# zhyever/PatchRefinerV2

Measured on AMD Instinct MI355X. Metric: 4K depth maps/sec (cai-mode r32), higher is better.
Workload: dtype bf16x3+f16f6; 1 GPU; v2_zoe_4k_r32; model=PatchRefinerPlus, cai_mode=r32, patches_per_frame=81, coarse_branch=ZoeDepth/DPT_BEiT_L_384, max_batch=41, streams=3, hip_graph=False, prefetch_next_coarse=True, frames=torch.rand, seeded, weights=synthetic (numpy PCG64 keyed by parameter name)

## Files before the change

patchrefinerv2_amd/csrc/conv3x3_f6.hip:

```cpp
#include <cstdlib>
#include <type_traits>

#include "igemm.h"
#include "conv3x3_gate_epi.h"

namespace prv2 {

namespace f6 {
constexpr int TH = 8, TW = 16, HW_ = TW + 2, HALO = (TH + 2) * HW_;
constexpr int PIX = 288;
constexpr int A_BYTES = HALO * PIX;
constexpr int ST_CHUNK = 1040, ST_DMAS = 6, ST_WAVE = ST_DMAS * ST_CHUNK;
constexpr int ST_BASE = 2 * A_BYTES;
constexpr int LDS_BYTES = ST_BASE + 8 * ST_WAVE;
constexpr int STEP_BYTES = 8 * 2 * 4 * 1024;
#ifndef F6_D
#define F6_D 4
#endif
constexpr int D = F6_D;
#ifndef F6_CV0
#define F6_CV0 2
#endif
#ifndef F6_CV1
#define F6_CV1 5
#endif
constexpr int CV_TAP0 = F6_CV0, CV_TAP1 = F6_CV1;
static_assert(LDS_BYTES <= 160 * 1024, "LDS budget");
static_assert(8 * ST_DMAS * 4 >= HALO, "staging covers the halo");
}

struct F6Params {
  const float* x;
  const char* w;
  const float* bias;
  const float* res;
  float* y;
  unsigned* range;
  int N, H, W, Cin, ldx, ldy, ld_res;
  long long x_bstride, y_bstride;
  float x_scale, out_scale;
  int relu_in, y_x2;
  long long* stamps;
};

typedef int i32x4 __attribute__((ext_vector_type(4)));
typedef int i32x8 __attribute__((ext_vector_type(8)));
typedef unsigned u32x6 __attribute__((ext_vector_type(6)));
typedef _Float16 f16x8 __attribute__((ext_vector_type(8)));

__device__ __forceinline__ u32x6 cvt_fp6(const f32x16& a, const f32x16& b, float scale) {
  u32x6 q;
  asm volatile("v_cvt_scalef32_2xpk16_fp6_f32 %0, %1, %2, %3" : "=&v"(q) : "v"(a), "v"(b), "v"(scale));
  return q;
}
__device__ __forceinline__ int e8m0_of(float m) {
  const int eb = (int)((__float_as_uint(m) >> 23) & 0xffu);
  return min(max(eb - 2, 1), 254);
}

__device__ __forceinline__ unsigned long long uniform64(unsigned long long v) {
  return (unsigned long long)(unsigned)__builtin_amdgcn_readfirstlane((int)(unsigned)v) |
         ((unsigned long long)(unsigned)__builtin_amdgcn_readfirstlane((int)(unsigned)(v >> 32)) << 32);
}

#ifndef F6_DBG_NOW
#define F6_LDW(dst, voff, sbase, imm) asm volatile("global_load_dwordx4 %0, %1, %2 offset:" #imm : "=v"(dst) : "v"(voff), "s"(sbase) : "memory")
#else
#define F6_LDW(dst, voff, sbase, imm) asm volatile("global_load_dwordx4 %0, %1, %2 offset:" #imm : "=v"(dst) : "v"(lane * 16), "s"(p.w) : "memory")
#endif

template <bool X2IN, class Epi>
__device__ __forceinline__ void f6_body(const F6Params& p, char* const smem, const int t_begin, const int per, const int K, Epi&& epi) {
  using namespace f6;
  const int tid = threadIdx.x, lane = tid & 63, wave = __builtin_amdgcn_readfirstlane(tid >> 6);
  const int m16 = lane & 15, g = lane >> 4;
  const unsigned lds0 = (unsigned)(size_t)smem;
  const int tiles_x = (p.W + TW - 1) / TW, tiles_xy = tiles_x * ((p.H + TH - 1) / TH);
  auto tile_of = [&](int k, int& n, int& y0, int& x0) {
    const int t = t_begin + k * per;
    n = t / tiles_xy;
    const int r = t - n * tiles_xy, ty = r / tiles_x;
    y0 = ty * TH;
    x0 = (r - ty * tiles_x) * TW;
  };

  constexpr unsigned OOB = 0x80000000u;
  i32x4 rsrc;
  rsrc.z = __builtin_amdgcn_readfirstlane((int)(unsigned)((((long long)p.H * p.W - 1) * p.ldx + p.Cin) * 4));
  rsrc.w = 0x00020000;
  unsigned hoff[ST_DMAS];
  auto set_loader = [&](int k) {
    int n, y0, x0;
    tile_of(k, n, y0, x0);
    const unsigned long long img_base = (unsigned long long)(size_t)(p.x + (long long)n * p.x_bstride);
    rsrc.x = __builtin_amdgcn_readfirstlane((int)(unsigned)img_base);
    rsrc.y = __builtin_amdgcn_readfirstlane((int)(unsigned)((img_base >> 32) & 0xffffu));
#pragma unroll
    for (int i = 0; i < ST_DMAS; ++i) {
      const int hp = (wave * ST_DMAS + i) * 4 + g;
      const int hy = hp / HW_, hx = hp - hy * HW_;
      const int iy = y0 - 1 + hy, ix = x0 - 1 + hx;
      const bool ok = hp < HALO && (unsigned)iy < (unsigned)p.H && (unsigned)ix < (unsigned)p.W;
      hoff[i] = ok ? (unsigned)(((iy * p.W + ix) * p.ldx + m16 * 4) * 4) : OOB;
    }
  };
  set_loader(0);
  const int nss = p.Cin >> 6, nsteps = nss * 9;
#ifdef F6_DBG_NODMA
  i32x4 dbg_sink;
#endif
  const unsigned st_wave = lds0 + ST_BASE + wave * ST_WAVE;
  auto dma_halo = [&](int ss) {
    const unsigned cofs = (unsigned)(ss * 256);
#pragma unroll
    for (int i = 0; i < ST_DMAS; ++i) {
      const unsigned dst = __builtin_amdgcn_readfirstlane(st_wave + i * ST_CHUNK);
      const unsigned voff = hoff[i] + cofs;
#ifndef F6_DBG_NODMA
      asm volatile("s_mov_b32 m0, %0\n\ts_nop 0\n\tbuffer_load_dwordx4 %1, %2, 0 offen lds" ::"s"(dst), "v"(voff), "s"(rsrc) : "memory");
#else
      asm volatile("buffer_load_dwordx4 %0, %1, %2, 0 offen" : "=v"(dbg_sink) : "v"(voff), "s"(rsrc) : "memory");
#endif
    }
  };
  const int lp = lane >> 1, cs = lane & 1, chp = wave * 24 + lp;
  const char* const st_rd = smem + ST_BASE + wave * ST_WAVE + (lp >> 2) * ST_CHUNK + (lp & 3) * 256 + cs * 128;
  const float xs = p.x_scale;
  const float relu_floor = p.relu_in ? 0.f : -__builtin_inff();
  float seen = 0.f;
  auto convert = [&](int wbuf) {
    if (lane < 48) {
      f32x16 a, b;
#pragma unroll
      for (int k = 0; k < 4; ++k) {
        f32x4 ta, tb;
        if constexpr (X2IN) {
          typedef unsigned u32x2v __attribute__((ext_vector_type(2)));
          const int q = k >> 1, h = k & 1;
          const u32x2v ah = *reinterpret_cast<const u32x2v*>(st_rd + 32 * q + 8 * h), al = *reinterpret_cast<const u32x2v*>(st_rd + 32 * q + 16 + 8 * h);
          const u32x2v bh = *reinterpret_cast<const u32x2v*>(st_rd + 64 + 32 * q + 8 * h), bl = *reinterpret_cast<const u32x2v*>(st_rd + 64 + 32 * q + 16 + 8 * h);
#pragma unroll
          for (int e = 0; e < 4; ++e) {
            const unsigned sh = (e & 1) ? 0u : 16u;
            ta[e] = __uint_as_float((ah[e >> 1] << sh) & 0xffff0000u) + __uint_as_float((al[e >> 1] << sh) & 0xffff0000u);
            tb[e] = __uint_as_float((bh[e >> 1] << sh) & 0xffff0000u) + __uint_as_float((bl[e >> 1] << sh) & 0xffff0000u);
          }
        } else {
          ta = *reinterpret_cast<const f32x4*>(st_rd + 16 * k);
          tb = *reinterpret_cast<const f32x4*>(st_rd + 64 + 16 * k);
        }
#pragma unroll
        for (int e = 0; e < 4; ++e) {
          a[4 * k + e] = fmaxf(ta[e], relu_floor) * xs;
          b[4 * k + e] = fmaxf(tb[e], relu_floor) * xs;
        }
// ... 71 lines not shown
#endif
  for (int ss = 0; ss < nss; ++ss) {
    const bool last_ss = ss + 1 == nss, more = !last_ss || k + 1 < K;
    const char* const xb = smem + ((k * nss + ss) & 1) * A_BYTES + xlane;
    auto read_item = [&](int it, int tap) {
      const int pp = it >> 3, a = it & 7, ky = tap / 3, kx = tap - 3 * ky;
      const char* q = xb + ((a + ky) * HW_ + kx) * PIX + (pp == 0 ? 0 : pp == 1 ? 64 : 128);
#ifdef F6_ABL_NOREAD
      if (k > 0 || ss > 0 || tap > 0 || it >= D) return;
#endif
      rlo[it % D] = *reinterpret_cast<const i32x4*>(q);
      if (pp == 2) rhi[it % D] = *reinterpret_cast<const i32x4*>(q + 64);
    };
    auto step = [&](auto tap_c) {
      constexpr int tap = decltype(tap_c)::value;
      constexpr int DM = tap == 0 ? ST_DMAS : 0;
      constexpr int DP = tap == 1 ? ST_DMAS : 0;
      const int s = ss * 9 + tap;
      const unsigned long long sb = uniform64(w_of(s + 1));
      if constexpr (tap == 0) {
#pragma unroll
        for (int it = 0; it < D - 1; ++it) read_item(it, 0);
      }
#pragma unroll
      for (int it = 0; it < 24; ++it) {
        const int pp = it >> 3, a = it & 7;
        if (it == 0) asm volatile("s_waitcnt vmcnt(%4)" : "+v"(wf0[0]), "+v"(wf0[1]), "+v"(wf1[0]), "+v"(wf1[1]) : "n"(6 + DP) : "memory");
        if (it == 8) asm volatile("s_waitcnt vmcnt(%2)" : "+v"(wf1[0]), "+v"(wf1[1]) : "n"(6 + DM) : "memory");
        if (it == 16) asm volatile("s_waitcnt vmcnt(%4)" : "+v"(wql[0]), "+v"(wqh[0]), "+v"(wql[1]), "+v"(wqh[1]) : "n"(4 + DM) : "memory");
        {
          const int nt = it + D - 1;
          if (nt < 24) read_item(nt, tap);
          else if (tap < 8) read_item(nt - 24, tap + 1);
        }
        __builtin_amdgcn_sched_barrier(0);
        if (pp == 0) {
          const f16x8 xf = __builtin_bit_cast(f16x8, rlo[it % D]);
          acc[a][0] = __builtin_amdgcn_mfma_f32_16x16x32_f16(__builtin_bit_cast(f16x8, wf0[0]), xf, acc[a][0], 0, 0, 0);
          acc[a][1] = __builtin_amdgcn_mfma_f32_16x16x32_f16(__builtin_bit_cast(f16x8, wf0[1]), xf, acc[a][1], 0, 0, 0);
        } else if (pp == 1) {
          const f16x8 xf = __builtin_bit_cast(f16x8, rlo[it % D]);
          acc[a][0] = __builtin_amdgcn_mfma_f32_16x16x32_f16(__builtin_bit_cast(f16x8, wf1[0]), xf, acc[a][0], 0, 0, 0);
          acc[a][1] = __builtin_amdgcn_mfma_f32_16x16x32_f16(__builtin_bit_cast(f16x8, wf1[1]), xf, acc[a][1], 0, 0, 0);
        } else {
          const i32x4 xl = rlo[it % D], xh = rhi[it % D];
          const i32x8 xq = {xl.x, xl.y, xl.z, xl.w, xh.x, xh.y, 0, 0};
          const i32x8 q0 = {wql[0].x, wql[0].y, wql[0].z, wql[0].w, wqh[0].x, wqh[0].y, 0, 0};
          const i32x8 q1 = {wql[1].x, wql[1].y, wql[1].z, wql[1].w, wqh[1].x, wqh[1].y, 0, 0};
          acc[a][0] = __builtin_amdgcn_mfma_scale_f32_16x16x128_f8f6f4(q0, xq, acc[a][0], 2, 2, 0, wqh[0].z, 0, xh.z);
          acc[a][1] = __builtin_amdgcn_mfma_scale_f32_16x16x128_f8f6f4(q1, xq, acc[a][1], 2, 2, 0, wqh[1].z, 0, xh.z);
        }
        __builtin_amdgcn_sched_barrier(0);
        if (it == 7) {
          F6_LOAD_F0(sb);
          if constexpr (tap == 0) {
            if (last_ss && k + 1 < K) set_loader(k + 1);
            dma_halo(last_ss ? (k + 1 < K ? 0 : ss) : ss + 1);
          }
#ifndef F6_ABL_NOCV
          if constexpr (tap == CV_TAP0) {
            if (more && wave < 4) convert((k * nss + ss + 1) & 1);
          }
          if constexpr (tap == CV_TAP1) {
            if (more && wave >= 4) convert((k * nss + ss + 1) & 1);
          }
#endif
        }
        if (it == 15) {
          F6_LOAD_F1(sb);
        }
        if (it == 23) F6_LOAD_Q(sb);
        __builtin_amdgcn_sched_barrier(0);
      }
    };
    step(std::integral_constant<int, 0>{});
    step(std::integral_constant<int, 1>{});
    step(std::integral_constant<int, 2>{});
    step(std::integral_constant<int, 3>{});
    step(std::integral_constant<int, 4>{});
    step(std::integral_constant<int, 5>{});
    step(std::integral_constant<int, 6>{});
    step(std::integral_constant<int, 7>{});
    step(std::integral_constant<int, 8>{});
    asm volatile("s_waitcnt lgkmcnt(0)\n\ts_barrier" ::: "memory");
  }
  {
#ifdef F6_STAMPS
    const long long st_b = __builtin_readcyclecounter();
#endif
    int n_img, y0, x0;
    tile_of(k, n_img, y0, x0);
    epi(n_img, y0, x0, acc, ((k * nss + nss - 1) & 1) * A_BYTES);
#ifdef F6_STAMPS
    const long long st_c = __builtin_readcyclecounter();
    st_main += st_b - st_a; st_epi += st_c - st_b;
#endif
  }
  }
  asm volatile("s_waitcnt vmcnt(0)" : "+v"(wf0[0]), "+v"(wf0[1]), "+v"(wf1[0]), "+v"(wf1[1]), "+v"(wql[0]), "+v"(wqh[0]), "+v"(wql[1]), "+v"(wqh[1])::"memory");
  if (p.range) {
    float m = seen;
#pragma unroll
    for (int o = 32; o > 0; o >>= 1) m = fmaxf(m, __shfl_xor(m, o, 64));
    if (lane == 0 && __float_as_uint(m) > __hip_atomic_load(p.range, __ATOMIC_RELAXED, __HIP_MEMORY_SCOPE_AGENT)) atomicMax(p.range, __float_as_uint(m));
  }
#ifdef F6_STAMPS
  if (p.stamps && lane == 0) {
    long long* o = p.stamps + ((long long)blockIdx.x * 8 + wave) * 8;
    o[0] = st_main; o[1] = st_epi; o[2] = K; o[3] = st_pro; o[4] = __builtin_readcyclecounter() - st_t0; o[5] = __builtin_amdgcn_s_memrealtime() - st_r0;
  }
#endif
}

__global__ void __launch_bounds__(512, 2) conv3x3_c256_f6_kernel(const F6Params p) {
  using namespace f6;
  __shared__ __attribute__((aligned(16))) char smem[LDS_BYTES];
  const int tiles_xy = ((p.W + TW - 1) / TW) * ((p.H + TH - 1) / TH), ntiles = p.N * tiles_xy;
  const int per = max((int)gridDim.x >> 3, 1), xcd = blockIdx.x & 7, jwg = blockIdx.x >> 3, chunk = (ntiles + 7) / 8;
  const int t_begin = xcd * chunk + jwg, t_end = min((xcd + 1) * chunk, ntiles);
  const int K = t_begin < t_end ? (t_end - t_begin + per - 1) / per : 0;
  if (K == 0) return;
  const int lane = threadIdx.x & 63, wave = __builtin_amdgcn_readfirstlane((int)threadIdx.x >> 6), m16 = lane & 15, g = lane >> 4;
  const int c0 = wave * 32 + g * 8;
  const float os = p.out_scale;
#ifndef F6_EPI_DIRECT
  constexpr int RP = 1040;
  const int tid = threadIdx.x, srow = tid >> 5, c8 = (tid & 31) * 8;
  f6_body<false>(p, smem, t_begin, per, K, [&](int n_img, int y0, int x0, f32x4 (&acc)[8][2], const int free_buf) {
    auto row_ptr = [&](int r) { return smem + (r < 48 ? ST_BASE + r * RP : free_buf + (r - 48) * RP); };
    f32x4 b0 = {0.f, 0.f, 0.f, 0.f}, b1 = b0;
    if (p.bias) {
      b0 = *reinterpret_cast<const f32x4*>(p.bias + c0);
      b1 = *reinterpret_cast<const f32x4*>(p.bias + c0 + 4);
    }
    const long long img_px = (long long)n_img * p.H * p.W;
    const __amdgpu_buffer_rsrc_t res_rs = __builtin_amdgcn_make_buffer_rsrc((void*)(p.res ? p.res + img_px * p.ld_res : p.x), 0,
                                                                            p.res ? (int)(((unsigned)(p.H * p.W - 1) * p.ld_res + 256) * 4u) : 0, 0x00020000);
    float* const ybase = p.y + (long long)n_img * p.y_bstride + c8;
#pragma unroll
    for (int h = 0; h < 2; ++h) {
      f32x4 r0[4], r1[4];
#pragma unroll
      for (int i = 0; i < 4; ++i) {
        const int iy = y0 + 4 * h + i, ixs = x0 + srow;
        const unsigned off = (iy < p.H && ixs < p.W) ? (unsigned)(((iy * p.W + ixs) * p.ld_res + c8) * 4) : 0x80000000u;
        r0[i] = __builtin_bit_cast(f32x4, __builtin_amdgcn_raw_buffer_load_b128(res_rs, off, 0, 0));
        r1[i] = __builtin_bit_cast(f32x4, __builtin_amdgcn_raw_buffer_load_b128(res_rs, off + 16, 0, 0));
      }
#pragma unroll
      for (int a = 0; a < 4; ++a) {
        char* q = row_ptr(a * TW + m16) + c0 * 4;
        *reinterpret_cast<f32x4*>(q) = acc[4 * h + a][0] * os + b0;
        *reinterpret_cast<f32x4*>(q + 16) = acc[4 * h + a][1] * os + b1;
        acc[4 * h + a][0] = acc[4 * h + a][1] = f32x4{0.f, 0.f, 0.f, 0.f};
      }
      asm volatile("s_waitcnt lgkmcnt(0)\n\ts_barrier" ::: "memory");
#pragma unroll
      for (int i = 0; i < 4; ++i) {
        const int iy = y0 + 4 * h + i, ixs = x0 + srow;
        const char* q = row_ptr(srow + 16 * i) + c8 * 4;
        const f32x4 v0 = *reinterpret_cast<const f32x4*>(q) + r0[i], v1 = *reinterpret_cast<const f32x4*>(q + 16) + r1[i];
#ifndef F6_DBG_NOEPI
        if (iy < p.H && ixs < p.W) {
          float* const dst = ybase + (long long)(iy * p.W + ixs) * p.ldy;
          if (p.y_x2) {
            bf16x4 h0, l0, h1, l1;
            split_bf16(v0, h0, l0);
            split_bf16(v1, h1, l1);
            const bf16x8 hv = __builtin_shufflevector(h0, h1, 0, 1, 2, 3, 4, 5, 6, 7), lv = __builtin_shufflevector(l0, l1, 0, 1, 2, 3, 4, 5, 6, 7);
            asm volatile("global_store_dwordx4 %0, %1, off\n\tglobal_store_dwordx4 %0, %2, off offset:16\n\ts_nop 1" ::"v"(dst), "v"(hv), "v"(lv) : "memory");
          } else {
            asm volatile("global_store_dwordx4 %0, %1, off\n\tglobal_store_dwordx4 %0, %2, off offset:16\n\ts_nop 1" ::"v"(dst), "v"(v0), "v"(v1) : "memory");
          }
        }
#endif
      }
      asm volatile("s_waitcnt lgkmcnt(0)\n\ts_barrier" ::: "memory");
    }
  });
#else
  f6_body<false>(p, smem, t_begin, per, K, [&](int n_img, int y0, int x0, f32x4 (&acc)[8][2], int) {
    f32x4 b0 = {0.f, 0.f, 0.f, 0.f}, b1 = b0;
    if (p.bias) {
      b0 = *reinterpret_cast<const f32x4*>(p.bias + c0);
      b1 = *reinterpret_cast<const f32x4*>(p.bias + c0 + 4);
    }
    const unsigned long long rb = (unsigned long long)(size_t)(p.res ? p.res + (long long)n_img * p.H * p.W * p.ld_res : p.x);
    i32x4 rr;
    rr.x = __builtin_amdgcn_readfirstlane((int)(unsigned)rb);
    rr.y = __builtin_amdgcn_readfirstlane((int)(unsigned)((rb >> 32) & 0xffffu));
    rr.z = __builtin_amdgcn_readfirstlane(p.res ? (int)(((unsigned)(p.H * p.W - 1) * p.ld_res + 256) * 4u) : 0);
    rr.w = 0x00020000;
    const int ix = x0 + m16;
    const unsigned voff = (unsigned)(((y0 * p.W + ix) * p.ld_res + c0) * 4);
    const int row = p.W * p.ld_res * 4;
    f32x4 r0[8], r1[8];
#pragma unroll
    for (int a = 0; a < 8; ++a) {
      const int so = __builtin_amdgcn_readfirstlane(a * row);
      asm volatile("buffer_load_dwordx4 %0, %2, %3, %4 offen\n\tbuffer_load_dwordx4 %1, %2, %3, %4 offen offset:16"
                   : "=&v"(r0[a]), "=&v"(r1[a]) : "v"(voff), "s"(rr), "s"(so) : "memory");
    }
    float* const ybase = p.y + (long long)n_img * p.y_bstride + c0;
#pragma unroll
    for (int a = 0; a < 8; ++a) {
      asm volatile("s_waitcnt vmcnt(%2)" : "+v"(r0[a]), "+v"(r1[a]) : "n"(2 * (7 - a)) : "memory");
      acc[a][0] = acc[a][0] * os + b0 + r0[a];
      acc[a][1] = acc[a][1] * os + b1 + r1[a];
    }
#pragma unroll
    for (int a = 0; a < 8; ++a) {
#ifndef F6_DBG_NOEPI
      if (y0 + a < p.H && ix < p.W) {
        const f32x4 v0 = acc[a][0], v1 = acc[a][1];
        float* const dst = ybase + (long long)((y0 + a) * p.W + ix) * p.ldy;
        if (p.y_x2) {
          bf16x4 h0, l0, h1, l1;
          split_bf16(v0, h0, l0);
          split_bf16(v1, h1, l1);
          const bf16x8 hv = __builtin_shufflevector(h0, h1, 0, 1, 2, 3, 4, 5, 6, 7), lv = __builtin_shufflevector(l0, l1, 0, 1, 2, 3, 4, 5, 6, 7);
          asm volatile("global_store_dwordx4 %0, %1, off\n\tglobal_store_dwordx4 %0, %2, off offset:16\n\ts_nop 1" ::"v"(dst), "v"(hv), "v"(lv) : "memory");
        } else {
          asm volatile("global_store_dwordx4 %0, %1, off\n\tglobal_store_dwordx4 %0, %2, off offset:16\n\ts_nop 1" ::"v"(dst), "v"(v0), "v"(v1) : "memory");
        }
      }
#endif
      acc[a][0] = acc[a][1] = f32x4{0.f, 0.f, 0.f, 0.f};
    }
  });
#endif
}

template <bool X2IN>
__global__ void __launch_bounds__(512, 2) conv3x3_c256_gate_f6_kernel(const GateConvParams gp) {
  using namespace f6;
  static_assert(LDS_BYTES >= g256::EPI_FLOATS * 4, "the C tile fits the main loop's LDS");
  __shared__ __attribute__((aligned(16))) char smem[LDS_BYTES];
  const IgemmParams& c = gp.c;
  F6Params p;
  p.x = c.x; p.w = reinterpret_cast<const char*>(c.w); p.bias = c.bias; p.res = nullptr; p.y = nullptr; p.range = gp.f6_range;
  p.N = c.N; p.H = c.H; p.W = c.W; p.Cin = c.Cin; p.ldx = c.ldx; p.ldy = c.ldy; p.ld_res = 0;
  p.x_bstride = c.x_bstride; p.y_bstride = c.y_bstride; p.x_scale = gp.f6_x_scale; p.out_scale = gp.f6_out_scale; p.relu_in = c.relu_in; p.y_x2 = 0;
  p.stamps = nullptr;
  int t = blockIdx.x;
  {
    const int ntiles = gridDim.x, q = ntiles >> 3, r = ntiles & 7, xcd = t & 7;
    t = (xcd < r ? xcd * (q + 1) : r * (q + 1) + (xcd - r) * q) + (t >> 3);
  }
  const int lane = threadIdx.x & 63, wave = __builtin_amdgcn_readfirstlane((int)threadIdx.x >> 6), m16 = lane & 15, g = lane >> 4;
  const int c0 = wave * 32 + g * 8;
  const float os = p.out_scale;
  PRV2_STAMP(0);
  PRV2_STAMP(1);
  PRV2_CLK_STAMP(0);
  f6_body<X2IN>(p, smem, t, 1, 1, [&](int n_img, int y0, int x0, f32x4 (&acc)[8][2], int) {
    asm volatile("s_waitcnt vmcnt(0) lgkmcnt(0)\n\ts_barrier" ::: "memory");
    PRV2_STAMP(2);
    c256_epilogue<PRV2_PREC_BF16X3, true, X2IN>(gp, reinterpret_cast<float*>(smem), n_img, y0, x0, [&](float* ct) {
      f32x4 b0 = {0.f, 0.f, 0.f, 0.f}, b1 = b0;
      if (c.bias) {
        b0 = *reinterpret_cast<const f32x4*>(c.bias + c0);
        b1 = *reinterpret_cast<const f32x4*>(c.bias + c0 + 4);
      }
#pragma unroll
      for (int a = 0; a < 8; ++a) {
        float* q = ct + (a * TW + m16) * g256::CLD + c0;
        *reinterpret_cast<f32x4*>(q) = acc[a][0] * os + b0;
        *reinterpret_cast<f32x4*>(q + 4) = acc[a][1] * os + b1;
      }
    });
  });
}

__global__ void __launch_bounds__(256) f6_pack_weight_kernel(const float* __restrict__ w, float w_scale, char* __restrict__ dst, int cin, int nsteps) {
  const int idx = blockIdx.x * blockDim.x + threadIdx.x;
  const int lane = idx & 63, j = (idx >> 6) & 1, wv = (idx >> 7) & 7, s = idx >> 10;
  if (s >= nsteps) return;
  const int ss = s / 9, tap = s - 9 * ss;
  const int r = lane & 15, g = lane >> 4;
  const int co = 32 * wv + 8 * (r >> 2) + 4 * j + (r & 3);
  const float* wr = w + (long long)co * cin * 9 + tap;
  char* o = dst + ((((long long)s * 8 + wv) * 2 + j) * 4) * 1024 + lane * 16;
#pragma unroll
  for (int part = 0; part < 2; ++part) {
    f16x8 h;
#pragma unroll
    for (int i = 0; i < 8; ++i) h[i] = (_Float16)(wr[(long long)(64 * ss + 32 * part + 8 * g + i) * 9] * w_scale);
    *reinterpret_cast<f16x8*>(o + part * 1024) = h;
  }
  f32x16 a, b;
  const int sl = g >> 1;
#pragma unroll
  for (int i = 0; i < 32; ++i) {
    const float v = wr[(long long)(64 * ss + 32 * sl + i) * 9] * w_scale;
    const float q = (g & 1) ? v : v - (float)(_Float16)v;
    if (i < 16) a[i] = q;
    else b[i - 16] = q;
  }
  float m = 0.f;
#pragma unroll
  for (int i = 0; i < 16; ++i) m = fmaxf(m, fmaxf(fabsf(a[i]), fabsf(b[i])));
  const int e = e8m0_of(m);
  const u32x6 q = cvt_fp6(a, b, __uint_as_float((unsigned)e << 23));
  typedef unsigned u32x4 __attribute__((ext_vector_type(4)));
  *reinterpret_cast<u32x4*>(o + 2 * 1024) = u32x4{q[0], q[1], q[2], q[3]};
  *reinterpret_cast<u32x4*>(o + 3 * 1024) = u32x4{q[4], q[5], (unsigned)e, 0u};
}

static inline bool aligned16(const void* q) { return (reinterpret_cast<uintptr_t>(q) & 15) == 0; }

static bool f6_shape_ok(const prv2_conv_desc* d) {
  return d->kh == 3 && d->kw == 3 && d->stride == 1 && d->pad == 1 && d->convt_k == 0 && !d->same_pad && d->cout == 256 && d->cin >= 64 &&
         d->cin % 64 == 0 && d->w >= f6::TW && (long long)d->h * d->w * d->ldx < (1LL << 29) && (long long)d->h * d->w * d->ldy < (1LL << 29);
}

}

using namespace prv2;

extern "C" int prv2_conv3x3_f6_supported(const prv2_conv_desc* d) { return d && f6_shape_ok(d) ? 1 : 0; }

extern "C" int64_t prv2_conv3x3_f6_weight_bytes(int32_t cout, int32_t cin) {
  return cout == 256 && cin >= 64 && cin % 64 == 0 ? (int64_t)(cin / 64) * 9 * f6::STEP_BYTES : 0;
}

extern "C" int prv2_pack_conv3x3_f6_weight(const float* w_src, float w_scale, void* w_packed, int32_t cout, int32_t cin, void* stream) {
  PRV2_REQUIRE(w_src && w_packed && aligned16(w_packed), "pack_conv3x3_f6_weight: null / unaligned pointer");
  PRV2_REQUIRE(prv2_conv3x3_f6_weight_bytes(cout, cin) > 0, "pack_conv3x3_f6_weight: 256 output channels, cin %% 64 == 0 (got %d -> %d)", cin, cout);
  PRV2_REQUIRE(w_scale > 0.f && (__builtin_bit_cast(unsigned, w_scale) & 0x7fffffu) == 0, "pack_conv3x3_f6_weight: w_scale is a power of two");
  const int nsteps = cin / 64 * 9;
  hipLaunchKernelGGL(f6_pack_weight_kernel, dim3((unsigned)(nsteps * 1024 / 256)), dim3(256), 0, (hipStream_t)stream, w_src, w_scale,
                     reinterpret_cast<char*>(w_packed), (int)cin, nsteps);
  PRV2_LAUNCH_CHECK("pack_conv3x3_f6_weight");
  return 0;
}

extern "C" int prv2_conv3x3_f6(const prv2_conv_desc* d, const float* x, const void* w_packed, const float* bias, const float* res, float x_scale,
                               float out_scale, uint32_t* range_word, float* y, void* stream) {
  PRV2_REQUIRE(d && x && w_packed && y, "conv3x3_f6: null pointer");
  PRV2_REQUIRE(f6_shape_ok(d), "conv3x3_f6: 3x3 s1 p1, cout 256, cin %% 64 == 0, width >= 16 (got %dx%d %d->%d k%d s%d)", d->h, d->w, d->cin, d->cout,
               d->kh, d->stride);
  PRV2_REQUIRE(d->act == PRV2_ACT_NONE && !(d->fmt & ~PRV2_FMT_Y_X2), "conv3x3_f6: no activation; the only format bit is PRV2_FMT_Y_X2");
  PRV2_REQUIRE(x_scale > 0.f && (__builtin_bit_cast(unsigned, x_scale) & 0x7fffffu) == 0 && out_scale > 0.f, "conv3x3_f6: x_scale is a power of two");
  F6Params p;
  memset(&p, 0, sizeof(p));
  p.x = x; p.w = reinterpret_cast<const char*>(w_packed); p.bias = bias; p.res = res; p.y = y; p.range = range_word;
  p.N = d->n; p.H = d->h; p.W = d->w; p.Cin = d->cin; p.ldx = d->ldx; p.ldy = d->ldy; p.ld_res = d->ld_res;
  p.x_bstride = d->x_bstride ? d->x_bstride : (long long)d->h * d->w * d->ldx;
  p.y_bstride = d->y_bstride ? d->y_bstride : (long long)d->h * d->w * d->ldy;
  p.x_scale = x_scale; p.out_scale = out_scale; p.relu_in = d->relu_in; p.y_x2 = (d->fmt & PRV2_FMT_Y_X2) != 0;
  PRV2_REQUIRE(d->n > 0 && d->h > 0 && d->ldx >= d->cin && d->ldx % 4 == 0 && aligned16(x) && p.x_bstride % 4 == 0, "conv3x3_f6: x layout");
  PRV2_REQUIRE(d->ldy >= d->cout && d->ldy % 4 == 0 && aligned16(y) && p.y_bstride % 4 == 0, "conv3x3_f6: y layout");
  PRV2_REQUIRE(!bias || aligned16(bias), "conv3x3_f6: bias alignment");
  PRV2_REQUIRE(!res || (d->ld_res >= d->cout && d->ld_res % 4 == 0 && aligned16(res) && (long long)d->h * d->w * d->ld_res < (1LL << 29)), "conv3x3_f6: res layout");
// ... 59 lines not shown
```

patchrefinerv2_amd/csrc/conv3x3_gate_epi.h:

```cpp
#pragma once
#include <cstdlib>
#include <type_traits>

#include "igemm.h"

namespace prv2 {

namespace g256 {
constexpr int BN = 256, TH = 8, TW = 16, HW_ = TW + 2;
constexpr int HALO = (TH + 2) * HW_;
constexpr int A_IT = (HALO * 8 + 511) / 512;
constexpr int A_IT2 = (HALO * 4 + 511) / 512;
constexpr int AROW = 160;
constexpr int A_BYTES = HALO * AROW, B_BYTES = BN * 128, NBUF = 3;
constexpr int CLD = BN + 4;
constexpr int ROWS = TH * TW;
constexpr int MAIN_BYTES = 2 * A_BYTES + NBUF * B_BYTES;
constexpr int EPI_FLOATS = ROWS * CLD + 2 * ROWS + 2 * BN;
constexpr int SMEM_FLOATS = MAIN_BYTES / 4 > EPI_FLOATS ? MAIN_BYTES / 4 : EPI_FLOATS;
static_assert(SMEM_FLOATS * 4 <= 160 * 1024, "LDS budget");
constexpr int NA = 4, NJ = 4, ND = 4;
}

__device__ __forceinline__ float sigmoid_fast(float v) {
// ... 270 lines not shown
  if (gp.y_x2) {
    constexpr int C8 = BN / 8, RPP8 = 512 / C8, NR8 = ROWS / RPP8;
    const int col8 = tid % C8;
    auto pix8 = [&](int i) {
      const int rr = tid / C8 + i * RPP8;
      return min(y0 + rr / TW, p.H - 1) * p.W + min(x0 + (rr & (TW - 1)), p.W - 1);
    };
    const __amdgpu_buffer_rsrc_t res_rs8 = __builtin_amdgcn_make_buffer_rsrc(
        (void*)(p.res ? p.res + (long long)n_img * p.H * p.W * p.ld_res : p.x), 0, p.res ? (int)(((unsigned)(p.H * p.W - 1) * p.ld_res + BN) * 4u) : 0,
        0x00020000);
    f32x4 rv8[NR8][2];
#pragma unroll
    for (int i = 0; i < NR8; ++i) {
      rv8[i][0] = __builtin_bit_cast(f32x4, __builtin_amdgcn_raw_buffer_load_b128(res_rs8, (pix8(i) * p.ld_res + col8 * 8) * 4, 0, 0));
      rv8[i][1] = __builtin_bit_cast(f32x4, __builtin_amdgcn_raw_buffer_load_b128(res_rs8, (pix8(i) * p.ld_res + col8 * 8 + 4) * 4, 0, 0));
    }
    float* const ybase8 = p.y + (long long)n_img * p.y_bstride + col8 * 8;
    dispatch_act(p.act, [&](auto act_c) {
#pragma unroll
      for (int i = 0; i < NR8; ++i) {
        const int rr = tid / C8 + i * RPP8;
        f32x4 v0 = *reinterpret_cast<const f32x4*>(&csm[rr * CLD + col8 * 8]), v1 = *reinterpret_cast<const f32x4*>(&csm[rr * CLD + col8 * 8 + 4]);
#pragma unroll
        for (int e = 0; e < 4; ++e) {
          v0[e] = act_apply_bf(v0[e], decltype(act_c)::value) + rv8[i][0][e];
          v1[e] = act_apply_bf(v1[e], decltype(act_c)::value) + rv8[i][1][e];
        }
        bf16x4 h0, l0, h1, l1;
        split_bf16(v0, h0, l0);
        split_bf16(v1, h1, l1);
        const bf16x8 hv = __builtin_shufflevector(h0, h1, 0, 1, 2, 3, 4, 5, 6, 7);
        const bf16x8 lv = __builtin_shufflevector(l0, l1, 0, 1, 2, 3, 4, 5, 6, 7);
        if (y0 + rr / TW < p.H && x0 + (rr & (TW - 1)) < p.W) {
          float* dst = ybase8 + (long long)pix8(i) * p.ldy;
          asm volatile("global_store_dwordx4 %0, %1, off\n\tglobal_store_dwordx4 %0, %2, off offset:16\n\ts_nop 1" ::"v"(dst), "v"(hv), "v"(lv) : "memory");
        }
      }
    });
    return;
  }
  constexpr int C4 = BN / 4, RPP = 512 / C4, NR = ROWS / RPP;
  const int col4 = tid % C4;
  auto pix_of = [&](int i) {
    const int rr = tid / C4 + i * RPP;
    return min(y0 + rr / TW, p.H - 1) * p.W + min(x0 + (rr & (TW - 1)), p.W - 1);
  };
  const __amdgpu_buffer_rsrc_t res_rs = __builtin_amdgcn_make_buffer_rsrc(
      (void*)(p.res ? p.res + (long long)n_img * p.H * p.W * p.ld_res : p.x), 0, p.res ? (int)(((unsigned)(p.H * p.W - 1) * p.ld_res + BN) * 4u) : 0,
      0x00020000);
  f32x4 rv[NR];
#pragma unroll
  for (int i = 0; i < NR; ++i) rv[i] = __builtin_bit_cast(f32x4, __builtin_amdgcn_raw_buffer_load_b128(res_rs, (pix_of(i) * p.ld_res + col4 * 4) * 4, 0, 0));
  float* const ybase = p.y + (long long)n_img * p.y_bstride + col4 * 4;
  auto store_rows = [&](auto act_c, auto ln_c) {
    constexpr bool LN = decltype(ln_c)::value;
    f32x4 lw = {1.f, 1.f, 1.f, 1.f}, lb = {0.f, 0.f, 0.f, 0.f};
    if constexpr (LN) {
      lw = *reinterpret_cast<const f32x4*>(ln_par + col4 * 4);
      lb = *reinterpret_cast<const f32x4*>(ln_par + BN + col4 * 4);
    }
#pragma unroll
    for (int i = 0; i < NR; ++i) {
      const int rr = tid / C4 + i * RPP;
      const f32x4 cv = *reinterpret_cast<const f32x4*>(&csm[rr * CLD + col4 * 4]);
      f32x4 ov;
#pragma unroll
      for (int e = 0; e < 4; ++e) {
        float t = cv[e];
        if constexpr (LN) t = (t - ln_stats[rr]) * ln_stats[ROWS + rr] * lw[e] + lb[e];
        ov[e] = act_apply_bf(t, decltype(act_c)::value) + rv[i][e];
      }
      if (y0 + rr / TW < p.H && x0 + (rr & (TW - 1)) < p.W) {
        float* dst = ybase + (long long)pix_of(i) * p.ldy;
        asm volatile("global_store_dwordx4 %0, %1, off\n\ts_nop 1" ::"v"(dst), "v"(ov) : "memory");
      }
    }
  };
  dispatch_act(p.act, [&](auto act_c) {
    if (has_ln) store_rows(act_c, std::true_type{});
    else store_rows(act_c, std::false_type{});
  });
}

}
```

Before: 7.731 depth maps/s.

## Specialize f6 gate-conv epilogue with register LayerNorm and prefetched pre-activation

Replaces the generic c256 gate epilogue for the f6 gate conv with a dedicated one. It applies bias and the pre-activation residual, then computes LayerNorm statistics in registers using a small LDS cross-wave reduction, instead of writing the whole fp32 C tile first. The pre-activation loads are issued through a tail hook before the final barrier so they overlap the end of the main loop, and the final barrier is skipped on the last step. The gate GEMM reads a bf16 hi/lo image from LDS with the gate weights prefetched in halves. This costs more register pressure (pv, wf, mv and rv arrays) and adds extra code paths.

```diff
diff --git a/patchrefinerv2_amd/csrc/conv3x3_f6.hip b/patchrefinerv2_amd/csrc/conv3x3_f6.hip
--- a/patchrefinerv2_amd/csrc/conv3x3_f6.hip
+++ b/patchrefinerv2_amd/csrc/conv3x3_f6.hip
@@ -69,8 +69,8 @@
 #define F6_LDW(dst, voff, sbase, imm) asm volatile("global_load_dwordx4 %0, %1, %2 offset:" #imm : "=v"(dst) : "v"(lane * 16), "s"(p.w) : "memory")
 #endif
 
-template <bool X2IN, class Epi>
-__device__ __forceinline__ void f6_body(const F6Params& p, char* const smem, const int t_begin, const int per, const int K, Epi&& epi) {
+template <bool X2IN, bool TAIL = false, class Epi, class Hook>
+__device__ __forceinline__ void f6_body(const F6Params& p, char* const smem, const int t_begin, const int per, const int K, Epi&& epi, Hook&& hook) {
   using namespace f6;
   const int tid = threadIdx.x, lane = tid & 63, wave = __builtin_amdgcn_readfirstlane(tid >> 6);
   const int m16 = lane & 15, g = lane >> 4;
@@ -308,9 +308,16 @@
     step(std::integral_constant<int, 6>{});
     step(std::integral_constant<int, 7>{});
     step(std::integral_constant<int, 8>{});
+    if (!(TAIL && last_ss)) asm volatile("s_waitcnt lgkmcnt(0)\n\ts_barrier" ::: "memory");
+  }
+  if constexpr (TAIL) {
+    int n_img, y0, x0;
+    tile_of(k, n_img, y0, x0);
+    hook(n_img, y0, x0);
     asm volatile("s_waitcnt lgkmcnt(0)\n\ts_barrier" ::: "memory");
   }
   {
+    if constexpr (TAIL) asm volatile("s_waitcnt vmcnt(0)" : "+v"(wf0[0]), "+v"(wf0[1]), "+v"(wf1[0]), "+v"(wf1[1]), "+v"(wql[0]), "+v"(wqh[0]), "+v"(wql[1]), "+v"(wqh[1])::"memory");
 #ifdef F6_STAMPS
     const long long st_b = __builtin_readcyclecounter();
 #endif
@@ -323,7 +330,7 @@
 #endif
   }
   }
-  asm volatile("s_waitcnt vmcnt(0)" : "+v"(wf0[0]), "+v"(wf0[1]), "+v"(wf1[0]), "+v"(wf1[1]), "+v"(wql[0]), "+v"(wqh[0]), "+v"(wql[1]), "+v"(wqh[1])::"memory");
+  if constexpr (!TAIL) asm volatile("s_waitcnt vmcnt(0)" : "+v"(wf0[0]), "+v"(wf0[1]), "+v"(wf1[0]), "+v"(wf1[1]), "+v"(wql[0]), "+v"(wqh[0]), "+v"(wql[1]), "+v"(wqh[1])::"memory");
   if (p.range) {
     float m = seen;
 #pragma unroll
@@ -336,6 +343,11 @@
     o[0] = st_main; o[1] = st_epi; o[2] = K; o[3] = st_pro; o[4] = __builtin_readcyclecounter() - st_t0; o[5] = __builtin_amdgcn_s_memrealtime() - st_r0;
   }
 #endif
+}
+
+template <bool X2IN, class Epi>
+__device__ __forceinline__ void f6_body(const F6Params& p, char* const smem, const int t_begin, const int per, const int K, Epi&& epi) {
+  f6_body<X2IN, false>(p, smem, t_begin, per, K, epi, [](int, int, int) {});
 }
 
 __global__ void __launch_bounds__(512, 2) conv3x3_c256_f6_kernel(const F6Params p) {
@@ -460,7 +472,7 @@
 template <bool X2IN>
 __global__ void __launch_bounds__(512, 2) conv3x3_c256_gate_f6_kernel(const GateConvParams gp) {
   using namespace f6;
-  static_assert(LDS_BYTES >= g256::EPI_FLOATS * 4, "the C tile fits the main loop's LDS");
+  static_assert(LDS_BYTES >= g256::F6_EPI_FLOATS * 4, "the operand image and the statistics areas fit the main loop's LDS");
   __shared__ __attribute__((aligned(16))) char smem[LDS_BYTES];
   const IgemmParams& c = gp.c;
   F6Params p;
@@ -473,29 +485,18 @@
     const int ntiles = gridDim.x, q = ntiles >> 3, r = ntiles & 7, xcd = t & 7;
     t = (xcd < r ? xcd * (q + 1) : r * (q + 1) + (xcd - r) * q) + (t >> 3);
   }
-  const int lane = threadIdx.x & 63, wave = __builtin_amdgcn_readfirstlane((int)threadIdx.x >> 6), m16 = lane & 15, g = lane >> 4;
-  const int c0 = wave * 32 + g * 8;
   const float os = p.out_scale;
   PRV2_STAMP(0);
   PRV2_STAMP(1);
   PRV2_CLK_STAMP(0);
-  f6_body<X2IN>(p, smem, t, 1, 1, [&](int n_img, int y0, int x0, f32x4 (&acc)[8][2], int) {
-    asm volatile("s_waitcnt vmcnt(0) lgkmcnt(0)\n\ts_barrier" ::: "memory");
-    PRV2_STAMP(2);
-    c256_epilogue<PRV2_PREC_BF16X3, true, X2IN>(gp, reinterpret_cast<float*>(smem), n_img, y0, x0, [&](float* ct) {
-      f32x4 b0 = {0.f, 0.f, 0.f, 0.f}, b1 = b0;
-      if (c.bias) {
-        b0 = *reinterpret_cast<const f32x4*>(c.bias + c0);
-        b1 = *reinterpret_cast<const f32x4*>(c.bias + c0 + 4);
-      }
-#pragma unroll
-      for (int a = 0; a < 8; ++a) {
-        float* q = ct + (a * TW + m16) * g256::CLD + c0;
-        *reinterpret_cast<f32x4*>(q) = acc[a][0] * os + b0;
-        *reinterpret_cast<f32x4*>(q + 4) = acc[a][1] * os + b1;
-      }
-    });
-  });
+  f32x4 pv[8][2];
+  f6_body<X2IN, true>(
+      p, smem, t, 1, 1,
+      [&](int n_img, int y0, int x0, f32x4 (&acc)[8][2], int) {
+        PRV2_STAMP(2);
+        c256_gate_epilogue_f6<X2IN>(gp, reinterpret_cast<float*>(smem), n_img, y0, x0, acc, pv, os);
+      },
+      [&](int n_img, int y0, int x0) { gate_f6_request_pre(gp, n_img, y0, x0, pv); });
 }
 
 __global__ void __launch_bounds__(256) f6_pack_weight_kernel(const float* __restrict__ w, float w_scale, char* __restrict__ dst, int cin, int nsteps) {
diff --git a/patchrefinerv2_amd/csrc/conv3x3_gate_epi.h b/patchrefinerv2_amd/csrc/conv3x3_gate_epi.h
--- a/patchrefinerv2_amd/csrc/conv3x3_gate_epi.h
+++ b/patchrefinerv2_amd/csrc/conv3x3_gate_epi.h
@@ -376,4 +376,318 @@
   });
 }
 
+namespace g256 {
+constexpr int RED_LD = 12;
+constexpr int F6_EPI_FLOATS = ROWS * CLD + 2 * ROWS * RED_LD;
 }
+
+__device__ __forceinline__ void gate_f6_request_pre(const GateConvParams& gp, const int n_img, const int y0, const int x0, f32x4 (&pv)[8][2]) {
+  using namespace g256;
+  const IgemmParams& p = gp.c;
+  const int lane = threadIdx.x & 63, wave = __builtin_amdgcn_readfirstlane((int)threadIdx.x >> 6), m16 = lane & 15, g = lane >> 4;
+  const __amdgpu_buffer_rsrc_t pre_rs = __builtin_amdgcn_make_buffer_rsrc(
+      (void*)(gp.pre ? gp.pre + (long long)n_img * p.H * p.W * gp.ld_pre : p.x), 0, gp.pre ? (int)(((unsigned)(p.H * p.W - 1) * gp.ld_pre + BN) * 4u) : 0, 0x00020000);
+  const int ix = min(x0 + m16, p.W - 1), c0 = wave * 32 + g * 8;
+#pragma unroll
+  for (int a = 0; a < 8; ++a) {
+    const int off = ((min(y0 + a, p.H - 1) * p.W + ix) * gp.ld_pre + c0) * 4;
+    pv[a][0] = __builtin_bit_cast(f32x4, __builtin_amdgcn_raw_buffer_load_b128(pre_rs, off, 0, 0));
+    pv[a][1] = __builtin_bit_cast(f32x4, __builtin_amdgcn_raw_buffer_load_b128(pre_rs, off + 16, 0, 0));
+  }
+}
+
+template <bool X2IN>
+__device__ __forceinline__ void c256_gate_epilogue_f6(const GateConvParams& gp, float* const csm, const int n_img, const int y0, const int x0, f32x4 (&acc)[8][2],
+                                                      const f32x4 (&pv)[8][2], const float os) {
+  using namespace g256;
+  typedef unsigned u32x4 __attribute__((ext_vector_type(4)));
+  const IgemmParams& p = gp.c;
+  const int tid = threadIdx.x, lane = tid & 63, wave = __builtin_amdgcn_readfirstlane(tid >> 6), m16 = lane & 15, g = lane >> 4;
+  const int c0 = wave * 32 + g * 8;
+  float* const red0 = csm + ROWS * CLD;
+  float* const red1 = red0 + ROWS * RED_LD;
+  constexpr int NA2 = 8, NJ2 = 2, KS2 = BN / 32;
+  {
+    f32x4 b0 = {0.f, 0.f, 0.f, 0.f}, b1 = b0;
+    if (p.bias) {
+      b0 = *reinterpret_cast<const f32x4*>(p.bias + c0);
+      b1 = *reinterpret_cast<const f32x4*>(p.bias + c0 + 4);
+    }
+#pragma unroll
+    for (int a = 0; a < 8; ++a) {
+      acc[a][0] = acc[a][0] * os + b0 + pv[a][0];
+      acc[a][1] = acc[a][1] * os + b1 + pv[a][1];
+    }
+  }
+  PRV2_STAMP(3);
+  u32x4 wf[KS2][NJ2][2];
+  const u32x4* const gw = reinterpret_cast<const u32x4*>(gp.gate_w) + lane;
+  auto request_gate_w = [&](int ks0, int ks1) {
+#pragma unroll
+    for (int ks = ks0; ks < ks1; ++ks)
+#pragma unroll
+      for (int j = 0; j < NJ2; ++j) {
+        wf[ks][j][0] = gw[gate_frag_index(BN, wave * NJ2 + j, ks, 0)];
+        wf[ks][j][1] = gw[gate_frag_index(BN, wave * NJ2 + j, ks, 1)];
+      }
+  };
+  request_gate_w(0, KS2 / 2);
+  const f32x4 lw0 = *reinterpret_cast<const f32x4*>(p.ln_w + c0), lw1 = *reinterpret_cast<const f32x4*>(p.ln_w + c0 + 4);
+  const f32x4 lb0 = *reinterpret_cast<const f32x4*>(p.ln_b + c0), lb1 = *reinterpret_cast<const f32x4*>(p.ln_b + c0 + 4);
+  auto row_sum = [&](float (&s)[8], float* const red) {
+#pragma unroll
+    for (int a = 0; a < 8; ++a) {
+      s[a] += __shfl_xor(s[a], 16, 64);
+      s[a] += __shfl_xor(s[a], 32, 64);
+    }
+    red[(g * TW + m16) * RED_LD + wave] = g == 0 ? s[0] : g == 1 ? s[1] : g == 2 ? s[2] : s[3];
+    red[((g + 4) * TW + m16) * RED_LD + wave] = g == 0 ? s[4] : g == 1 ? s[5] : g == 2 ? s[6] : s[7];
+    asm volatile("s_waitcnt lgkmcnt(0)\n\ts_barrier" ::: "memory");
+#pragma unroll
+    for (int a = 0; a < 8; ++a) {
+      const float* q = red + (a * TW + m16) * RED_LD;
+      const f32x4 t0 = *reinterpret_cast<const f32x4*>(q), t1 = *reinterpret_cast<const f32x4*>(q + 4);
+      s[a] = ((t0.x + t0.y) + (t0.z + t0.w)) + ((t1.x + t1.y) + (t1.z + t1.w));
+    }
+  };
+  float mean[8], rstd[8];
+#pragma unroll
+  for (int a = 0; a < 8; ++a) {
+    const f32x4 v0 = acc[a][0], v1 = acc[a][1];
+    mean[a] = ((v0.x + v0.y) + (v0.z + v0.w)) + ((v1.x + v1.y) + (v1.z + v1.w));
+  }
+  row_sum(mean, red0);
+#pragma unroll
+  for (int a = 0; a < 8; ++a) {
+    mean[a] = mean[a] / (float)BN;
+    const f32x4 d0 = acc[a][0] - mean[a], d1 = acc[a][1] - mean[a];
+    rstd[a] = ((d0.x * d0.x + d0.y * d0.y) + (d0.z * d0.z + d0.w * d0.w)) + ((d1.x * d1.x + d1.y * d1.y) + (d1.z * d1.z + d1.w * d1.w));
+  }
+  row_sum(rstd, red1);
+#pragma unroll
+  for (int a = 0; a < 8; ++a) rstd[a] = 1.0f / sqrtf(rstd[a] / (float)BN + p.ln_eps);
+  PRV2_STAMP(4);
+  {
+    const float act_floor = p.act == PRV2_ACT_RELU ? 0.f : -__builtin_inff();
+#pragma unroll
+    for (int a = 0; a < 8; ++a) {
+      f32x4 v0 = (acc[a][0] - mean[a]) * rstd[a] * lw0 + lb0;
+      f32x4 v1 = (acc[a][1] - mean[a]) * rstd[a] * lw1 + lb1;
+#pragma unroll
+      for (int e = 0; e < 4; ++e) {
+        v0[e] = fmaxf(v0[e], act_floor);
+        v1[e] = fmaxf(v1[e], act_floor);
+      }
+      bf16x4 h0, l0, h1, l1;
+      split_bf16(v0, h0, l0);
+      split_bf16(v1, h1, l1);
+      float* q = csm + (a * TW + m16) * CLD + c0;
+      *reinterpret_cast<bf16x8*>(q) = __builtin_shufflevector(h0, h1, 0, 1, 2, 3, 4, 5, 6, 7);
+      *reinterpret_cast<bf16x8*>(q + 4) = __builtin_shufflevector(l0, l1, 0, 1, 2, 3, 4, 5, 6, 7);
+      acc[a][0] = acc[a][1] = f32x4{0.f, 0.f, 0.f, 0.f};
+    }
+  }
+  request_gate_w(KS2 / 2, KS2);
+  asm volatile("s_waitcnt lgkmcnt(0)\n\ts_barrier" ::: "memory");
+  PRV2_STAMP(5);
+  const long long img_m = (long long)n_img * p.H * p.W;
+  const unsigned img_px = (unsigned)(p.H * p.W - 1);
+  const __amdgpu_buffer_rsrc_t mul_rs = __builtin_amdgcn_make_buffer_rsrc(
+      (void*)(p.mul ? p.mul + img_m * p.ld_mul : p.x), 0, p.mul ? (int)((img_px * p.ld_mul + BN) * 4u) : 0, 0x00020000);
+  const __amdgpu_buffer_rsrc_t res_rs = __builtin_amdgcn_make_buffer_rsrc(
+      (void*)(p.res ? p.res + img_m * p.ld_res : p.x), 0, p.res ? (int)((img_px * p.ld_res + BN) * 4u) : 0, 0x00020000);
+  const bool has_mul = p.mul != nullptr;
+  const int m16r = (m16 >= 4 && m16 < 12) ? 2 * (m16 - 4) : 2 * (m16 & 3) + 1 + (m16 >= 12 ? 8 : 0);
+  f32x4 acc2[NA2][NJ2];
+#pragma unroll
+  for (int a = 0; a < NA2; ++a)
+#pragma unroll
+    for (int j = 0; j < NJ2; ++j) acc2[a][j] = f32x4{0.f, 0.f, 0.f, 0.f};
+#ifndef PRV2_ABL_GATE_LDS_STORE
+  const int chb = wave * 32 + 4 * g;
+  const int pxc = min(x0 + m16r, p.W - 1);
+  auto pix_of = [&](int a) { return min(y0 + a, p.H - 1) * p.W + pxc; };
+  f32x4 mv[NA2][NJ2];
+  f32x4 rv[NA2][NJ2];
+#pragma unroll
+  for (int ks = 0; ks < KS2; ++ks) {
+    if (ks == KS2 - 3) {
+#pragma unroll
+      for (int a = 0; a < NA2; ++a)
+#pragma unroll
+        for (int j = 0; j < NJ2; ++j) {
+          if constexpr (X2IN) {
+            typedef unsigned u32x2 __attribute__((ext_vector_type(2)));
+            const int off = (pix_of(a) * p.ld_mul + wave * 32 + 16 * j + 8 * (g >> 1)) * 4 + 8 * (g & 1);
+            const u32x2 hh = __builtin_bit_cast(u32x2, __builtin_amdgcn_raw_buffer_load_b64(mul_rs, off, 0, 0));
+            const u32x2 ll = __builtin_bit_cast(u32x2, __builtin_amdgcn_raw_buffer_load_b64(mul_rs, off + 16, 0, 0));
+            mv[a][j] = __builtin_bit_cast(f32x4, u32x4{hh[0], hh[1], ll[0], ll[1]});
+          } else {
+            mv[a][j] = __builtin_bit_cast(f32x4, __builtin_amdgcn_raw_buffer_load_b128(mul_rs, (pix_of(a) * p.ld_mul + chb + 16 * j) * 4, 0, 0));
+          }
+        }
+    }
+#pragma unroll
+    for (int h = 0; h < 2; ++h) {
+      bf16x8 xh[4], xl[4];
+#pragma unroll
+      for (int a = 0; a < 4; ++a) {
+        const float* q = csm + ((4 * h + a) * TW + m16r) * CLD + ks * 32 + 8 * g;
+        xh[a] = *reinterpret_cast<const bf16x8*>(q);
+        xl[a] = *reinterpret_cast<const bf16x8*>(q + 4);
+      }
+#pragma unroll
+      for (int j = 0; j < NJ2; ++j) {
+        const bf16x8 wh = __builtin_bit_cast(bf16x8, wf[ks][j][0]);
+        const bf16x8 wl = __builtin_bit_cast(bf16x8, wf[ks][j][1]);
+#pragma unroll
+        for (int a = 0; a < 4; ++a) acc2[4 * h + a][j] = __builtin_amdgcn_mfma_f32_16x16x32_bf16(wh, xl[a], acc2[4 * h + a][j], 0, 0, 0);
+#pragma unroll
+        for (int a = 0; a < 4; ++a) acc2[4 * h + a][j] = __builtin_amdgcn_mfma_f32_16x16x32_bf16(wl, xh[a], acc2[4 * h + a][j], 0, 0, 0);
+#pragma unroll
+        for (int a = 0; a < 4; ++a) acc2[4 * h + a][j] = __builtin_amdgcn_mfma_f32_16x16x32_bf16(wh, xh[a], acc2[4 * h + a][j], 0, 0, 0);
+      }
+    }
+  }
+  PRV2_STAMP(6);
+#pragma unroll
+  for (int a = 0; a < NA2; ++a)
+#pragma unroll
+    for (int j = 0; j < NJ2; ++j)
+      rv[a][j] = __builtin_bit_cast(f32x4, __builtin_amdgcn_raw_buffer_load_b128(res_rs, (pix_of(a) * p.ld_res + chb + 16 * j) * 4, 0, 0));
+  PRV2_STAMP(7);
+  f32x4 gb[NJ2];
+#pragma unroll
+  for (int j = 0; j < NJ2; ++j) gb[j] = gp.gate_bias ? *reinterpret_cast<const f32x4*>(gp.gate_bias + chb + 16 * j) : f32x4{0.f, 0.f, 0.f, 0.f};
+  float* const ybase = p.y + (long long)n_img * p.y_bstride + chb;
+  const bool col_in = x0 + m16r < p.W;
+#pragma unroll
+  for (int a = 0; a < NA2; ++a) {
+    float* const dst = ybase + (long long)pix_of(a) * p.ldy;
+#pragma unroll
+    for (int j = 0; j < NJ2; ++j) {
+      f32x4 mf;
+      if constexpr (X2IN) {
+        const u32x4 m = __builtin_bit_cast(u32x4, mv[a][j]);
+        mf[0] = __builtin_bit_cast(float, m[0] << 16) + __builtin_bit_cast(float, m[2] << 16);
+        mf[1] = __builtin_bit_cast(float, m[0] & 0xffff0000u) + __builtin_bit_cast(float, m[2] & 0xffff0000u);
+        mf[2] = __builtin_bit_cast(float, m[1] << 16) + __builtin_bit_cast(float, m[3] << 16);
+        mf[3] = __builtin_bit_cast(float, m[1] & 0xffff0000u) + __builtin_bit_cast(float, m[3] & 0xffff0000u);
+      } else {
+        bf16x4 mh, ml;
+        split_bf16(mv[a][j], mh, ml);
+        mf = __builtin_convertvector(mh, f32x4) + __builtin_convertvector(ml, f32x4);
+      }
+      f32x4 ov;
+#pragma unroll
+      for (int e = 0; e < 4; ++e) ov[e] = (has_mul ? mf[e] : 1.0f) * sigmoid_fast(acc2[a][j][e] + gb[j][e]) + rv[a][j][e];
+      if (col_in && y0 + a < p.H) {
+        float* d2 = dst + 16 * j;
+        asm volatile("global_store_dwordx4 %0, %1, off\n\ts_nop 1" ::"v"(d2), "v"(ov) : "memory");
+      }
+    }
+  }
+#else
+  const int grow = g == 0 ? 1 : (g == 3 ? 9 : 8 * (g - 1));
+  constexpr int NC = X2IN ? 8 : 4, NV = NC / 4;
+  constexpr int CG = BN / NC, RPP = 512 / CG, NR = ROWS / RPP;
+  const int colg = tid % CG;
+  auto pix_of = [&](int i) {
+    const int rr = tid / CG + i * RPP;
+    return min(y0 + rr / TW, p.H - 1) * p.W + min(x0 + (rr & (TW - 1)), p.W - 1);
+  };
+  f32x4 mv[NR][NV], rv[NR][NV];
+#pragma unroll
+  for (int ks = 0; ks < KS2; ++ks) {
+    if (ks == KS2 - 3) {
+#pragma unroll
+      for (int i = 0; i < NR; ++i)
+#pragma unroll
+        for (int v = 0; v < NV; ++v)
+          mv[i][v] = __builtin_bit_cast(f32x4, __builtin_amdgcn_raw_buffer_load_b128(mul_rs, (pix_of(i) * p.ld_mul + colg * NC + 4 * v) * 4, 0, 0));
+    }
+#pragma unroll
+    for (int h = 0; h < 2; ++h) {
+      bf16x8 xh[4], xl[4];
+#pragma unroll
+      for (int a = 0; a < 4; ++a) {
+        const float* q = csm + ((4 * h + a) * TW + m16r) * CLD + ks * 32 + 8 * g;
+        xh[a] = *reinterpret_cast<const bf16x8*>(q);
+        xl[a] = *reinterpret_cast<const bf16x8*>(q + 4);
+      }
+#pragma unroll
+      for (int j = 0; j < NJ2; ++j) {
+        const bf16x8 wh = __builtin_bit_cast(bf16x8, wf[ks][j][0]);
+        const bf16x8 wl = __builtin_bit_cast(bf16x8, wf[ks][j][1]);
+#pragma unroll
+        for (int a = 0; a < 4; ++a) acc2[4 * h + a][j] = __builtin_amdgcn_mfma_f32_16x16x32_bf16(xl[a], wh, acc2[4 * h + a][j], 0, 0, 0);
+#pragma unroll
+        for (int a = 0; a < 4; ++a) acc2[4 * h + a][j] = __builtin_amdgcn_mfma_f32_16x16x32_bf16(xh[a], wl, acc2[4 * h + a][j], 0, 0, 0);
+#pragma unroll
+        for (int a = 0; a < 4; ++a) acc2[4 * h + a][j] = __builtin_amdgcn_mfma_f32_16x16x32_bf16(xh[a], wh, acc2[4 * h + a][j], 0, 0, 0);
+      }
+    }
+  }
+  PRV2_STAMP(6);
+#pragma unroll
+  for (int i = 0; i < NR; ++i)
+#pragma unroll
+    for (int v = 0; v < NV; ++v)
+      rv[i][v] = __builtin_bit_cast(f32x4, __builtin_amdgcn_raw_buffer_load_b128(res_rs, (pix_of(i) * p.ld_res + colg * NC + 4 * v) * 4, 0, 0));
+  asm volatile("s_waitcnt lgkmcnt(0)\n\ts_barrier" ::: "memory");
+#pragma unroll
+  for (int j = 0; j < NJ2; ++j) {
+    const int col = wave * 32 + j * 16 + m16;
+#pragma unroll
+    for (int a = 0; a < NA2; ++a)
+#pragma unroll
+      for (int e = 0; e < 4; ++e) csm[(a * TW + grow + 2 * e) * CLD + col] = acc2[a][j][e];
+  }
+  asm volatile("s_waitcnt lgkmcnt(0)\n\ts_barrier" ::: "memory");
+  PRV2_STAMP(7);
+  f32x4 gb[NV];
+#pragma unroll
+  for (int v = 0; v < NV; ++v) gb[v] = gp.gate_bias ? *reinterpret_cast<const f32x4*>(gp.gate_bias + colg * NC + 4 * v) : f32x4{0.f, 0.f, 0.f, 0.f};
+  float* const ybase = p.y + (long long)n_img * p.y_bstride + colg * NC;
+#pragma unroll
+  for (int i = 0; i < NR; ++i) {
+    const int rr = tid / CG + i * RPP;
+    f32x4 mf[NV];
+    if constexpr (X2IN) {
+      const u32x4 hh = __builtin_bit_cast(u32x4, mv[i][0]), ll = __builtin_bit_cast(u32x4, mv[i][NV - 1]);
+#pragma unroll
+      for (int v = 0; v < NV; ++v) {
+        mf[v][0] = __builtin_bit_cast(float, hh[2 * v] << 16) + __builtin_bit_cast(float, ll[2 * v] << 16);
+        mf[v][1] = __builtin_bit_cast(float, hh[2 * v] & 0xffff0000u) + __builtin_bit_cast(float, ll[2 * v] & 0xffff0000u);
+        mf[v][2] = __builtin_bit_cast(float, hh[2 * v + 1] << 16) + __builtin_bit_cast(float, ll[2 * v + 1] << 16);
+        mf[v][3] = __builtin_bit_cast(float, hh[2 * v + 1] & 0xffff0000u) + __builtin_bit_cast(float, ll[2 * v + 1] & 0xffff0000u);
+      }
+    } else {
+      bf16x4 mh, ml;
+      split_bf16(mv[i][0], mh, ml);
+      mf[0] = __builtin_convertvector(mh, f32x4) + __builtin_convertvector(ml, f32x4);
+    }
+    const bool inside = y0 + rr / TW < p.H && x0 + (rr & (TW - 1)) < p.W;
+    float* dst = ybase + (long long)pix_of(i) * p.ldy;
+#pragma unroll
+    for (int v = 0; v < NV; ++v) {
+      const f32x4 cv = *reinterpret_cast<const f32x4*>(&csm[rr * CLD + colg * NC + 4 * v]);
+      f32x4 ov;
+#pragma unroll
+      for (int e = 0; e < 4; ++e) ov[e] = (has_mul ? mf[v][e] : 1.0f) * sigmoid_fast(cv[e] + gb[v][e]) + rv[i][v][e];
+      if (inside) {
+        float* d2 = dst + 4 * v;
+        asm volatile("global_store_dwordx4 %0, %1, off\n\ts_nop 1" ::"v"(d2), "v"(ov) : "memory");
+      }
+    }
+  }
+#endif
+  PRV2_STAMP(8);
+#ifdef PRV2_GATE_STAMPS
+  asm volatile("s_waitcnt vmcnt(0)" ::: "memory");
+  PRV2_STAMP(9);
+  PRV2_CLK_STAMP(1);
+#endif
+}
+
+}
```

New measurement: 7.702 depth maps/s. No clear change (-0.4%).
